# johannes-graeter/limo

Hardware: NVIDIA H100
Metric: BA windows/s (30 KF, 3k LM, 40k obs) (higher is better)
Workload: dtype f64

## Files before the change

### limo_b200/csrc/kba_api.cu

```cuda
#include <algorithm>
#include <atomic>
#include <chrono>
#include <cstdio>
#include <cstdlib>
#include <cstring>
#include <string>
#include <thread>
#include <vector>

#include <cuda_runtime.h>

#include "kba_b200.h"
#include "kba_kernels.h"

using namespace kba;

static thread_local std::string g_last_error;
static thread_local bool g_force_host_pack = false;
static int fail(int code, const std::string& msg) {
    g_last_error = msg;
    return code;
}
#define CU(call)                                                                                              \
    do {                                                                                                      \
// ... 576 lines not shown
        d.scale_kf0 = w[i].scale_kf0; d.scale_kf1 = w[i].scale_kf1;
        d.scale_weight = w[i].scale_weight; d.scale_value = w[i].scale_value;
        const bool planes = w[i].n_gp > 0 || w[i].plane_reg_weight > 0;
        const int rows = (planes ? 10 : 6) * w[i].n_kf + 1;
        max_rows = std::max(max_rows, rows);
        d.nr_cap = ((rows + 63) / 64) * 64;
        d.plane_reg_weight = w[i].plane_reg_weight; d.plane_dist_fixed = w[i].plane_dist_fixed;
        d.s_off = soff;
        soff += (long long)d.nr_cap * d.nr_cap;
        nr_cap_max = std::max(nr_cap_max, d.nr_cap);
        kf += w[i].n_kf; cam += w[i].n_cam; lm += w[i].n_lm; obs += w[i].n_obs; chunks += d.n_chunks; gp += w[i].n_gp;
        bd.max_obs = std::max(bd.max_obs, w[i].n_obs); bd.max_lm = std::max(bd.max_lm, w[i].n_lm);
        bd.max_kf = std::max(bd.max_kf, w[i].n_kf); bd.max_gp = std::max(bd.max_gp, w[i].n_gp);
    }
    if (obs > 2000000000LL) { b->release(); delete b; return fail(KBA_ERR_CAPACITY, "batch exceeds 2^31 observations"); }
    if (nr_cap_max > 640) {
        b->release();
        delete b;
        return fail(KBA_ERR_CAPACITY, "reduced system larger than 640 rows (106 keyframes, or 63 with ground-plane blocks)");
    }
    bd.tot_kf = kf; bd.tot_cam = cam; bd.tot_lm = lm; bd.tot_obs = obs; bd.tot_chunks = (int)chunks; bd.tot_gp = gp;
    bd.tot_groups = (int)groups;
    bd.nr_cap_max = nr_cap_max;
    b->lc.nr_cap_max = nr_cap_max;
    b->lc.sm_count = h->sm_count;
    {
        const int nb = nr_cap_max / 64, pairs = nb * (nb + 1) / 2;
        int max_chunks = 1;
        for (auto& d : b->desc_h) max_chunks = std::max(max_chunks, d.n_chunks);
        int p = std::min(16, (6 * h->sm_count + n_windows * pairs - 1) / (n_windows * pairs));
        b->lc.small_syrk = (max_rows <= 184);
        if (b->lc.small_syrk) p = (h->sm_count + n_windows - 1) / n_windows;
        bd.p_split = std::max(1, std::min(p, max_chunks));
        const char* fe = std::getenv("KBA_FUSED");
        bd.fused = (b->lc.small_syrk && bd.max_kf <= kFusedMaxKf && !(fe && std::atoi(fe) == 0)) ? 1 : 0;
        if (const char* pe = std::getenv("KBA_P_SPLIT")) { if (std::atoi(pe) > 0) p = std::atoi(pe); }
        if (bd.fused) bd.p_split = std::max(1, std::min(p, max_groups));
        else if (std::getenv("KBA_P_SPLIT")) bd.p_split = std::max(1, std::min(p, max_chunks));
        b->lc.fused_slots = (max_rows_free <= 176) ? 6 : 7;
    }
    bd.cost_parts = std::max((bd.max_obs + 255) / 256, (bd.max_obs / 16 + bd.max_lm / 32 + 4 + 7) / 8);
    { const char* le = std::getenv("KBA_LINEARIZE"); b->lc.lin_fused = !(le && std::atoi(le) == 0); }
    { const char* le = std::getenv("KBA_LIN_GRID"); if (le) b->lc.lin_grid = std::max(-1, std::atoi(le)); }
    { const char* le = std::getenv("KBA_BS_GRID"); if (le) b->lc.bs_grid = std::max(-1, std::atoi(le)); }
    {
        auto knob = [](const char* name, int dflt) { const char* e = std::getenv(name); return e ? std::atoi(e) : dflt; };
        bd.eval_tiles_jac = std::max(1, knob("KBA_EVAL_TILES_JAC", 8));
        bd.eval_tiles_cost = std::max(1, knob("KBA_EVAL_TILES_COST", 8));
        bd.eval_min_blocks = knob("KBA_EVAL_MIN_BLOCKS", 2);
        bd.eval_cs = knob("KBA_EVAL_CS", 0);
        bd.solve_row_major = knob("KBA_SOLVE_ROW_MAJOR", 0);
        bd.solve_tiled = (nr_cap_max <= 192 && !bd.solve_row_major) ? 1 : 0;
        const int split_dflt = (!bd.solve_tiled && n_windows <= 16) ? std::max(1, std::min(32, h->sm_count / n_windows)) : 0;
        bd.solve_split = bd.solve_tiled ? 0 : knob("KBA_SOLVE_SPLIT", split_dflt);
    }
    bd.bs_parts = (bd.max_lm + 15) / 16;
    {
        const char* pe = std::getenv("KBA_DEVICE_PACK");
        b->device_pack = bd.fused && !g_force_host_pack && bd.max_lm <= pack_max_landmarks() && !(pe && std::atoi(pe) == 0);
    }
    const bool hp = !b->device_pack;
    int bad = 0;
    bad |= b->desc.alloc(n_windows, true);
    bad |= b->pose0.alloc(7 * kf, true); bad |= b->plane0.alloc(4 * kf, true); bad |= b->kf_fixed.alloc(kf, true);
    bad |= b->cam.alloc(kCamStride * cam, true);
    bad |= b->lm0.alloc(3 * lm, hp); bad |= b->lm_weight.alloc(lm, hp); bad |= b->lm_ptr.alloc(lm + n_windows, hp);
    bad |= b->obs_kf.alloc(obs, hp); bad |= b->obs_cam.alloc(obs, hp); bad |= b->obs_lm.alloc(obs, hp);
    bad |= b->obs_u.alloc(obs, hp); bad |= b->obs_v.alloc(obs, hp); bad |= b->obs_d.alloc(obs, hp);
    bad |= b->kf_ptr.alloc(kf + n_windows, hp); bad |= b->pm_lm.alloc(obs, hp); bad |= b->pm_cam.alloc(obs, hp);
    bad |= b->pm_u.alloc(obs, hp); bad |= b->pm_v.alloc(obs, hp); bad |= b->pm_d.alloc(obs, hp);
    bad |= b->chunk_lm0.alloc(chunks, hp); bad |= b->chunk_lm1.alloc(chunks, hp);
    bad |= b->chunk_k0.alloc(chunks, hp); bad |= b->chunk_k1.alloc(chunks, hp);
    bad |= b->lm_orig.alloc(lm, hp); bad |= b->obs_rank.alloc(obs, hp);
    if (hp) bad |= b->obs_orig.alloc(obs, true);
    bad |= b->grp_k0.alloc(groups, hp); bad |= b->grp_k1.alloc(groups, hp);
    if (b->device_pack) {
        bad |= b->r_lm_ptr.alloc(lm + n_windows, true); bad |= b->r_obs_kf.alloc(obs, true); bad |= b->r_obs_cam.alloc(obs, true);
        bad |= b->r_obs_u.alloc(obs, true); bad |= b->r_obs_v.alloc(obs, true); bad |= b->r_obs_d.alloc(obs, true);
        bad |= b->r_lm_pos.alloc(3 * lm, true); bad |= b->r_lm_weight.alloc(lm, true); bad |= b->r_gp_lm.alloc(gp, true);
        bad |= b->lm_user.alloc(3 * lm, true); bad |= b->rej_user.alloc(lm, true);
        bad |= b->dev_alloc(&b->raw.lm_inv, lm);
    }
    bad |= b->dev_alloc(&bd.grp_t0, groups); bad |= b->dev_alloc(&bd.grp_t1, groups); bad |= b->dev_alloc(&bd.grp_rs, groups);
    bad |= b->dev_alloc(&bd.lin_tile, (size_t)(obs / 16) + (size_t)(lm / 32) + 4 * (size_t)n_windows + 4);
#ifdef KBA_PROF
    bad |= b->dev_alloc(&bd.prof, 16);
    if (!bad) cudaMemset(bd.prof, 0, 16 * sizeof(unsigned long long));
#endif
    bad |= b->dev_alloc(&bd.rt[0], (size_t)kPoseStride * kf); bad |= b->dev_alloc(&bd.rt[1], (size_t)kPoseStride * kf);
    {
        bd.panel_cap = 0;
        bd.vpanel = nullptr;
        bad |= b->dev_alloc(&bd.chunk_poff, chunks); bad |= b->dev_alloc(&bd.chunk_rs, chunks);
    }
    bad |= b->dev_alloc(&bd.chunk_t0, chunks); bad |= b->dev_alloc(&bd.chunk_t1, chunks); bad |= b->dev_alloc(&bd.obs_row, obs);
    bad |= b->state.alloc(n_windows, true); bad |= b->log.alloc((size_t)n_windows * kIterLogCap, true);
    for (int q = 0; q < 2; ++q) { bad |= b->pose_out[q].alloc(7 * kf, true); bad |= b->lm_out[q].alloc(3 * lm, hp); }
    bad |= b->lm_active.alloc(lm, hp); bad |= b->n_active.alloc(1, true); bad |= b->jac_obs.alloc(1, true);
    bad |= b->plane_out[0].alloc(4 * kf, true); bad |= b->plane_out[1].alloc(4 * kf, true);
    bad |= b->gp_lm.alloc(gp, hp); bad |= b->gp_kf.alloc(gp, true); bad |= b->gp_weight.alloc(gp, true); bad |= b->gp_of_lm.alloc(lm, hp); bad |= b->gp_shared.alloc(gp, hp);
    bad |= b->dev_alloc(&bd.gp_lin, 14 * gp); bad |= b->dev_alloc(&bd.vgp, 30 * gp);
    bad |= b->dev_alloc(&bd.gp_cost_x, n_windows); bad |= b->dev_alloc(&bd.gp_cost_c, n_windows);
    bad |= b->dev_alloc(&bd.off_pose, kf); bad |= b->dev_alloc(&bd.off_dir, kf); bad |= b->dev_alloc(&bd.off_dist, kf);
    bad |= b->dev_alloc(&bd.bkf, 27 * kf);
    bad |= b->dev_alloc(&bd.scale_f, (size_t)n_windows * nr_cap_max); bad |= b->dev_alloc(&bd.lambda_f, (size_t)n_windows * nr_cap_max);
    bad |= b->dev_alloc(&bd.grad_f, (size_t)n_windows * nr_cap_max); bad |= b->dev_alloc(&bd.delta_f, (size_t)n_windows * nr_cap_max);
    bad |= b->dev_alloc(&bd.lm_scale, 3 * lm); bad |= b->dev_alloc(&bd.lm_linv, 6 * lm); bad |= b->dev_alloc(&bd.lm_z, 3 * lm);
    bad |= b->dev_alloc(&bd.lm_g, 3 * lm); bad |= b->dev_alloc(&bd.lm_lambda, 3 * lm); bad |= b->dev_alloc(&bd.trim_val, 3 * lm);
    bad |= b->dev_alloc(&bd.trim_reject, lm);
    bad |= b->dev_alloc(&bd.res, 3 * obs); bad |= b->dev_alloc(&bd.jp, 18 * obs);
    if (!bd.fused) bad |= b->dev_alloc(&bd.jl, 9 * obs);
    else { bad |= b->dev_alloc(&bd.vobs, 18 * obs); bad |= b->dev_alloc(&bd.lm_run, lm); }
    bad |= b->dev_alloc(&bd.cost_part_x, (size_t)n_windows * bd.cost_parts); bad |= b->dev_alloc(&bd.cost_part_c, (size_t)n_windows * bd.cost_parts);
    bad |= b->dev_alloc(&bd.bs_part, (size_t)n_windows * bd.bs_parts * 4);
    bad |= b->dev_alloc(&bd.sred, (size_t)soff * bd.p_split); bad |= b->dev_alloc(&bd.amat, (size_t)soff);
    bad |= b->dev_alloc(&bd.chol_w, (size_t)n_windows * 32 * 32); bad |= b->dev_alloc(&bd.chol_invd, (size_t)n_windows * nr_cap_max);
    if (bad) {
        const std::string msg = std::string("device/pinned allocation failed: ") + cudaGetErrorString(cudaGetLastError());
        b->release(); delete b;
        return fail(KBA_ERR_CUDA, msg);
    }
    bd.desc = b->desc.d; bd.state = b->state.d; bd.log = b->log.d;
    bd.pose0 = b->pose0.d; bd.plane0 = b->plane0.d; bd.pose[0] = b->pose_out[0].d; bd.pose[1] = b->pose_out[1].d;
    bd.kf_fixed = b->kf_fixed.d; bd.cam = b->cam.d;
    bd.lm0 = b->lm0.d; bd.lm[0] = b->lm_out[0].d; bd.lm[1] = b->lm_out[1].d; bd.lm_weight = b->lm_weight.d;
    bd.lm_active = b->lm_active.d; bd.lm_ptr = b->lm_ptr.d;
    bd.obs_kf = b->obs_kf.d; bd.obs_cam = b->obs_cam.d; bd.obs_lm = b->obs_lm.d;
    bd.obs_u = b->obs_u.d; bd.obs_v = b->obs_v.d; bd.obs_d = b->obs_d.d;
    bd.kf_ptr = b->kf_ptr.d; bd.pm_lm = b->pm_lm.d; bd.pm_cam = b->pm_cam.d; bd.pm_u = b->pm_u.d; bd.pm_v = b->pm_v.d; bd.pm_d = b->pm_d.d;
    bd.chunk_lm0 = b->chunk_lm0.d; bd.chunk_lm1 = b->chunk_lm1.d; bd.chunk_k0 = b->chunk_k0.d; bd.chunk_k1 = b->chunk_k1.d;
    bd.lm_orig = b->lm_orig.d;
    bd.obs_rank = b->obs_rank.d;
    bd.grp_k0 = b->grp_k0.d; bd.grp_k1 = b->grp_k1.d;
    bd.plane[0] = b->plane_out[0].d; bd.plane[1] = b->plane_out[1].d;
    bd.gp_lm = b->gp_lm.d; bd.gp_kf = b->gp_kf.d; bd.gp_weight = b->gp_weight.d; bd.gp_of_lm = b->gp_of_lm.d; bd.gp_shared = b->gp_shared.d;
    bd.n_active = b->n_active.d;
    bd.jac_obs = b->jac_obs.d;
    if (b->device_pack) {
        PackRaw& r = b->raw;
        r.lm_ptr = b->r_lm_ptr.d; r.obs_kf = b->r_obs_kf.d; r.obs_cam = b->r_obs_cam.d;
        r.obs_u = b->r_obs_u.d; r.obs_v = b->r_obs_v.d; r.obs_d = b->r_obs_d.d;
        r.lm_pos = b->r_lm_pos.d; r.lm_weight = b->r_lm_weight.d; r.gp_lm = b->r_gp_lm.d; r.obs_orig = nullptr;
    }
    {
        cudaError_t e = cudaMemset(bd.jac_obs, 0, sizeof(unsigned long long));
        if (e == cudaSuccess) e = cudaEventCreate(&b->ev_a);
        if (e == cudaSuccess) e = cudaEventCreate(&b->ev_b);
        if (e == cudaSuccess) e = cudaEventCreateWithFlags(&b->ev_poll, (h->blocking_sync ? cudaEventBlockingSync : 0) | cudaEventDisableTiming);
        if (e == cudaSuccess) e = cudaEventCreateWithFlags(&b->ev_poll2, (h->blocking_sync ? cudaEventBlockingSync : 0) | cudaEventDisableTiming);
        if (e == cudaSuccess && b->loop_pass.alloc(1, true)) e = cudaErrorMemoryAllocation;
        if (e == cudaSuccess) e = configure_kernels(nr_cap_max);
        if (e == cudaSuccess && b->device_pack) e = configure_pack();
        if (e != cudaSuccess) { b->release(); delete b; return fail(KBA_ERR_CUDA, cudaGetErrorString(e)); }
    }
    *out = b;
    const int rc = kba_batch_upload(b, n_windows, w);
    if (rc != KBA_OK) { b->release(); delete b; *out = nullptr; }
    return rc;
}

int kba_batch_upload(kba_batch* b, int32_t n_windows, const kba_window* w) {
    if (!b || !w || n_windows != b->bd.n_win) return fail(KBA_ERR_BAD_ARG, "bad argument to kba_batch_upload");
    CU(cudaSetDevice(b->h->device));
    for (int i = 0; i < n_windows; ++i) {
        const WinDesc& d = b->desc_h[i];
        std::string why;
// ... 695 lines not shown
```

### limo_b200/csrc/kba_device.cuh

```cuda
#pragma once
#include <cstdint>
#include <cuda_runtime.h>

namespace kba {

constexpr int kMaxKf = 128;
constexpr int kMaxCam = 8;
constexpr int kPoseStride = 12;
constexpr int kCamStride = 16;
constexpr int kIterLogCap = 160;
constexpr int kFusedMaxKf = 32;

struct WinDesc {
    int n_kf, n_cam, n_lm, n_obs, n_gp;
    int kf_off, cam_off, lm_off, obs_off, gp_off;
    int chunk_off, n_chunks;
    int grp_off, n_groups;
    int scale_kf0, scale_kf1;
    double scale_weight, scale_value;
    double plane_reg_weight;
    int plane_dist_fixed, landmarks_fixed;
    int speed_kf, pad0;
    double speed_weight, speed_dt;
    double speed_v_before[3];
// ... 55 lines not shown
    double* plane0;
    double* pose[2];
    double* rt[2];
    double* plane[2];
    uint8_t* kf_fixed;
    int* off_pose;
    int* off_dir;
    int* off_dist;
    double* bkf;
    double* scale_f;
    double* cam;
    double* lm0;
    double* lm[2];
    double* lm_weight;
    uint8_t* lm_active;
    uint8_t* lm_active0;
    int* lm_ptr;
    double* lm_scale;
    double* lm_linv;
    double* lm_z;
    double* lm_g;
    double* lm_lambda;
    double* trim_val;
    uint8_t* trim_reject;
    int* obs_kf;
    int* obs_cam;
    int* obs_lm;
    int* obs_rank;
    float* obs_u, *obs_v, *obs_d;
    int* kf_ptr;
    int* pm_lm;
    int* pm_cam;
    float* pm_u, *pm_v, *pm_d;
    double* res;
    double* jp;
    double* jl;
    double* vpanel;
    long long panel_cap;
    int* chunk_poff;
    int* chunk_rs;
    double* cost_part_x;
    double* cost_part_c;
    int cost_parts;
    int sharded;
    int lm_begin, lm_total;
    int shard_rank, shard_world;
    double* xs;
    double* x_send;
    double* x_recv;
    double* trim_send;
    double* trim_glob;
    uint8_t* reject_glob;
    int precision;
    int solve_row_major;
    int solve_tiled;
    int solve_split;
    double* chol_w;
    double* chol_invd;
    int eval_tiles_jac, eval_tiles_cost, eval_min_blocks;
    int eval_cs;
    double* bs_part;
    int bs_parts;
    int nr_cap_max;
    double* sred;
    int p_split;
    double* delta_f;
    double* lambda_f;
    double* grad_f;
    double* amat;
    int* chunk_lm0;
    int* chunk_lm1;
    int* chunk_k0;
    int* chunk_k1;
    int* chunk_t0;
    int* chunk_t1;
    int* obs_row;
    int* lm_orig;
    int tot_chunks;
    int fused;
    int* grp_k0;
    int* grp_k1;
    int* grp_t0;
    int* grp_t1;
    int* grp_rs;
    double* vobs;
    int4* lm_run;
    int lin1;
    int2* lin_tile;
    unsigned long long* prof;
    int tot_groups;
    int* n_active;
    unsigned long long* jac_obs;
    int* gp_lm;
    int* gp_kf;
    double* gp_weight;
    int* gp_of_lm;
    int* gp_shared;
    double* gp_lin;
    double* vgp;
    double* gp_cost_x;
    double* gp_cost_c;
};

struct SolveParams {
    double gp_huber, gp_quantile;
    double depth_thres, reprojection_thres, depth_quantile, reprojection_quantile;
    double function_tolerance, gradient_tolerance, parameter_tolerance;
    double initial_radius, max_radius, min_radius, min_relative_decrease, min_lm_diagonal, max_lm_diagonal;
    int trim_solver_iterations, final_solver_iterations, min_residual_groups, max_consecutive_invalid_steps;
    double max_solver_time;
};

__device__ __forceinline__ unsigned long long global_timer_ns() {
    unsigned long long t;
    asm volatile("mov.u64 %0, %%globaltimer;" : "=l"(t));
    return t;
}

template <typename T>
__host__ __device__ inline void quat_to_rot(const T* q, T* R) {
    const T w = q[0], x = q[1], y = q[2], z = q[3];
    const T tx = 2 * x, ty = 2 * y, tz = 2 * z;
    const T twx = tx * w, twy = ty * w, twz = tz * w, txx = tx * x, txy = ty * x, txz = tz * x;
    const T tyy = ty * y, tyz = tz * y, tzz = tz * z;
    R[0] = 1 - (tyy + tzz); R[1] = txy - twz;       R[2] = txz + twy;
    R[3] = txy + twz;       R[4] = 1 - (txx + tzz); R[5] = tyz - twx;
    R[6] = txz - twy;       R[7] = tyz + twx;       R[8] = 1 - (txx + tyy);
}

__host__ __device__ inline void pose_plus(const double* p, const double* d, double* o) {
    const double nd = sqrt(d[0] * d[0] + d[1] * d[1] + d[2] * d[2]);
    if (nd > 0.0) {
        const double s = sin(nd) / nd, c = cos(nd);
        const double q0 = c, q1 = s * d[0], q2 = s * d[1], q3 = s * d[2];
        o[0] = q0 * p[0] - q1 * p[1] - q2 * p[2] - q3 * p[3];
        o[1] = q0 * p[1] + q1 * p[0] + q2 * p[3] - q3 * p[2];
        o[2] = q0 * p[2] - q1 * p[3] + q2 * p[0] + q3 * p[1];
        o[3] = q0 * p[3] + q1 * p[2] - q2 * p[1] + q3 * p[0];
    } else {
        o[0] = p[0]; o[1] = p[1]; o[2] = p[2]; o[3] = p[3];
    }
    o[4] = p[4] + d[3]; o[5] = p[5] + d[4]; o[6] = p[6] + d[5];
}

template <typename T, bool kCost = true>
__device__ inline void cauchy(T b, T w, T s, T& half_rho, T& sqrt_rho1) {
    const T sum = T(1) + s / b;
    half_rho = kCost ? T(0.5) * w * b * log(sum) : T(0);
    sqrt_rho1 = sqrt(w / sum);
}

template <typename T, bool kM, bool kCost = true>
__device__ __forceinline__ bool eval_factored(const T* __restrict__ pose, const T* __restrict__ cam, const T p[3], T u, T v,
                                              T d, T wt, T b_repr, T b_depth, T r[3], T m[9], T a[3], T& half_rho_sum,
                                              T raw[2]) {
    a[0] = pose[0] * p[0] + pose[1] * p[1] + pose[2] * p[2];
    a[1] = pose[3] * p[0] + pose[4] * p[1] + pose[5] * p[2];
    a[2] = pose[6] * p[0] + pose[7] * p[1] + pose[8] * p[2];
    const T x0 = a[0] + pose[9], x1 = a[1] + pose[10], x2 = a[2] + pose[11];
    const T c0 = cam[0] * x0 + cam[1] * x1 + cam[2] * x2 + cam[9];
    const T c1 = cam[3] * x0 + cam[4] * x1 + cam[5] * x2 + cam[10];
    const T c2 = cam[6] * x0 + cam[7] * x1 + cam[8] * x2 + cam[11];
    if (!(fabs(c2) >= T(0.01))) return false;
    const bool has_d = d > T(0);
    const T rd = has_d ? c2 - d : T(0);
    const T f = cam[12], iz = T(1) / c2;
// ... 202 lines not shown
```

### limo_b200/csrc/kba_kernels.cu

```cuda
#include "kba_device.cuh"
#include "kba_kernels.h"
#include "kba_regularisers.cuh"
#include "kba_prep.cuh"
#include "kba_linearize.cuh"

#include <cfloat>
#include <cstdio>
#include <cstdlib>
#include <cmath>
#include <type_traits>

namespace kba {

constexpr int kBeginThreads = 1024;
__global__ void __launch_bounds__(kBeginThreads) k_solve_begin(BatchDev bd, SolveParams sp) {
    const int w = blockIdx.x;
    WinState& st = bd.state[w];
    if (st.phase != PH_SOLVE_BEGIN) return;
    const WinDesc wd = bd.desc[w];
    __shared__ int s_has[kMaxKf];
    __shared__ int s_plane[kMaxKf];
    __shared__ int s_cnt[3];
    __shared__ int s_tile_chunk[513];
    for (int k = threadIdx.x; k < wd.n_kf; k += blockDim.x) { s_has[k] = 0; s_plane[k] = 0; }
// ... 38 lines not shown
            bd.off_pose[wd.kf_off + k] = var ? n : -1;
            if (var) n += 6;
            const bool pl = (s_plane[k] || chain) && !fixed;
            bd.off_dir[wd.kf_off + k] = pl ? n : -1;
            if (pl) n += 3;
            const bool pd = pl && !wd.plane_dist_fixed;
            bd.off_dist[wd.kf_off + k] = pd ? n : -1;
            if (pd) n += 1;
        }
        if (chain) n_reg = 3 * (wd.n_kf - 1) + wd.n_kf;
        st.n_f = n;
        st.nr = (n + 1 + 7) & ~7;
        st.radius = sp.initial_radius;
        st.decrease_factor = 2.0;
        st.iteration = 0;
        st.num_invalid = 0;
        st.last_successful = 0;
        st.need_linearize = 1;
        st.iter0 = 1;
        st.eval_failed = 0;
        st.solve_failed = 0;
        st.max_iter = st.is_final ? sp.final_solver_iterations
                                  : (st.retried ? 3 * sp.trim_solver_iterations : sp.trim_solver_iterations);
        SolveSummary& s = st.solves[st.solve_index];
        s.initial_cost = s.final_cost = 0.0;
        s.num_iterations = 0; s.num_successful_steps = 0; s.termination = 1;
        s.num_landmarks = s_cnt[0];
        s.num_residual_blocks = s_cnt[1] + s_cnt[2] + n_reg + (wd.scale_weight > 0 ? 1 : 0) + (wd.speed_weight > 0 ? 1 : 0);
        st.t_solve_start = global_timer_ns();
        st.phase = PH_ITERATE;
    }
    __syncthreads();
    for (int o = threadIdx.x; o < wd.n_obs; o += blockDim.x) {
        const size_t oo = (size_t)wd.obs_off + o;
        const bool act = bd.lm_active[wd.lm_off + bd.obs_lm[oo]];
        bd.obs_row[oo] = act ? bd.off_pose[wd.kf_off + bd.obs_kf[oo]] : -1;
    }
    for (int c = threadIdx.x; c < (bd.fused ? 0 : wd.n_chunks); c += blockDim.x) {
        int r0 = 1 << 30, r1 = -1;
        for (int k = bd.chunk_k0[wd.chunk_off + c]; k <= bd.chunk_k1[wd.chunk_off + c]; ++k) {
            const int off = bd.off_pose[wd.kf_off + k], od = bd.off_dir[wd.kf_off + k], oz = bd.off_dist[wd.kf_off + k];
            if (off >= 0) { r0 = min(r0, off); r1 = max(r1, off + 6); }
            if (od >= 0) { r0 = min(r0, od); r1 = max(r1, od + 3); }
            if (oz >= 0) { r0 = min(r0, oz); r1 = max(r1, oz + 1); }
        }
        bd.chunk_t0[wd.chunk_off + c] = (r1 < 0) ? 0 : r0 / 8;
        bd.chunk_t1[wd.chunk_off + c] = (r1 < 0) ? 0 : (r1 + 7) / 8;
    }
    if (bd.fused) {
        __syncthreads();
        for (int j = threadIdx.x; j < wd.n_lm; j += blockDim.x) {
            const int o0 = lm_ptr[j], o1 = lm_ptr[j + 1];
            int n_start = 0, n_valid = 0, bad = 0, a = 0, row_a = 0, prev = -2;
            for (int o = o0; o < o1; ++o) {
                const size_t oo = (size_t)wd.obs_off + o;
                const int r = bd.obs_row[oo];
                if (r >= 0) {
                    ++n_valid;
                    if (prev < 0) { if (n_start++ == 0) { a = o - o0; row_a = r; } }
                    else if (r != prev + 6) bad = 1;
                    if (bd.obs_rank[oo] != 0) bad = 1;
                }
                prev = r;
            }
            int4 run = make_int4(0, 0, 0, 0);
            if (n_valid > 0) run = (bad || n_start != 1) ? make_int4(0, -1, 0, 0) : make_int4(a, n_valid, row_a, 0);
            bd.lm_run[wd.lm_off + j] = run;
        }
    }
    if (bd.fused) build_lin_tiles(bd, wd, st, w, s_tile_chunk);
    if (bd.fused) {
        const int trhs = st.n_f >> 3;
        for (int c = threadIdx.x; c < wd.n_groups; c += blockDim.x) {
            int r0 = 1 << 30, r1 = -1;
            for (int k = bd.grp_k0[wd.grp_off + c]; k <= bd.grp_k1[wd.grp_off + c]; ++k) {
                const int off = bd.off_pose[wd.kf_off + k], od = bd.off_dir[wd.kf_off + k], oz = bd.off_dist[wd.kf_off + k];
                if (off >= 0) { r0 = min(r0, off); r1 = max(r1, off + 6); }
                if (od >= 0) { r0 = min(r0, od); r1 = max(r1, od + 3); }
                if (oz >= 0) { r0 = min(r0, oz); r1 = max(r1, oz + 1); }
            }
            const int t0 = (r1 < 0) ? 0 : (r0 / 16) * 2, t1 = (r1 < 0) ? 0 : ((r1 + 15) / 16) * 2;
            int rows = 0;
            if (t1 > t0) rows = 8 * (t1 - t0) + ((trhs >= t0 && trhs < t1) ? 0 : 8);
            bd.grp_t0[wd.grp_off + c] = t0;
            bd.grp_t1[wd.grp_off + c] = t1;
            bd.grp_rs[wd.grp_off + c] = rows;
        }
    }
    if (!bd.fused) {
        __syncthreads();
        if (threadIdx.x == 0) {
            const int trhs = st.n_f >> 3;
            int poff = 0;
            for (int c = 0; c < wd.n_chunks; ++c) {
                const int t0 = bd.chunk_t0[wd.chunk_off + c], t1 = bd.chunk_t1[wd.chunk_off + c];
                int rs = 0;
                if (t1 > t0) {
                    const int rows = 8 * (t1 - t0) + ((trhs >= t0 && trhs < t1) ? 0 : 8);
                    rs = ((rows - 4 + 15) / 16) * 16 + 4;
                }
                bd.chunk_rs[wd.chunk_off + c] = rs;
                bd.chunk_poff[wd.chunk_off + c] = poff;
                poff += 96 * rs;
            }
        }
    }
}

__global__ void __launch_bounds__(256) k_panel_zero(BatchDev bd) {
    const int w = blockIdx.y;
    if (bd.fused || bd.state[w].phase != PH_SOLVE_BEGIN || bd.desc[w].landmarks_fixed) return;
    double2* p = reinterpret_cast<double2*>(bd.vpanel + bd.desc[w].panel_off);
    const long long n2 = bd.panel_cap / 2;
    for (long long i = (long long)blockIdx.x * blockDim.x + threadIdx.x; i < n2; i += (long long)gridDim.x * blockDim.x)
        p[i] = make_double2(0.0, 0.0);
}

template <bool kJac, int kMinBlocks, typename TLin, bool kJl = true, bool kCs = false>
__global__ void __launch_bounds__(256, kMinBlocks) k_eval_obs(BatchDev bd, SolveParams sp, int tiles) {
    const int w = blockIdx.y;
    WinState& st = bd.state[w];
    const WinDesc& wd = bd.desc[w];
    const int n_obs = wd.n_obs, obs_off = wd.obs_off, lm_off = wd.lm_off;
    if (st.phase != PH_ITERATE) return;
    if (kJac && !st.need_linearize) return;
    if (!kJac && st.solve_failed) return;
    __shared__ __align__(16) double s_pose[kMaxKf * kPoseStride];
    __shared__ __align__(16) double s_cam[kMaxCam * kCamStride];
    __shared__ __align__(8) uint64_t s_bar;
    __shared__ double s_red[8];
    __shared__ int s_cnt[8];
    constexpr bool kF32 = sizeof(TLin) == 4;
    __shared__ float s_pose_f[kF32 ? kMaxKf * kPoseStride : 1];
    __shared__ float s_cam_f[kF32 ? kMaxCam * kCamStride : 1];
    const int buf = kJac ? st.cur : 1 - st.cur;
    const double* __restrict__ lm_buf = bd.lm[buf];
    const int i0 = blockIdx.x * tiles * 256 + threadIdx.x;
    int idx_b = (i0 < n_obs) ? bd.obs_lm[(size_t)obs_off + i0] : -1;
    int idx_a = (tiles > 1 && i0 + 256 < n_obs) ? bd.obs_lm[(size_t)obs_off + i0 + 256] : -1;
    int L = -1, kfi = 0, cami = 0, row = -1;
    float u = 0.f, v = 0.f, d = 0.f;
    double p0 = 0, p1 = 0, p2 = 0, wgt = 0;
    unsigned char act = 0;
    if (idx_b >= 0) {
        const size_t o = (size_t)obs_off + i0;
        L = lm_off + idx_b;
        kfi = bd.obs_kf[o]; cami = bd.obs_cam[o];
        if (kJac) row = bd.obs_row[o];
        u = bd.obs_u[o]; v = bd.obs_v[o]; d = bd.obs_d[o];
        p0 = lm_buf[3 * (size_t)L]; p1 = lm_buf[3 * (size_t)L + 1]; p2 = lm_buf[3 * (size_t)L + 2];
        wgt = bd.lm_weight[L];
        act = bd.lm_active[L];
    }
    stage_window_bulk(wd, bd.rt[buf], bd.cam, s_pose, s_cam, &s_bar);
    if (kF32) {
        for (int i = threadIdx.x; i < wd.n_kf * kPoseStride; i += blockDim.x) s_pose_f[i] = (float)s_pose[i];
        for (int i = threadIdx.x; i < wd.n_cam * kCamStride; i += blockDim.x) s_cam_f[i] = (float)s_cam[i];
        __syncthreads();
    }
    double cost = 0.0;
    int done = 0;
#pragma unroll 1
    for (int t = 0; t < tiles; ++t) {
        const int i_n = i0 + (t + 1) * 256;
        int Ln = -1, kfn = 0, camn = 0, rown = -1;
        float un = 0.f, vn = 0.f, dn = 0.f;
        double q0 = 0, q1 = 0, q2 = 0, wn = 0;
        unsigned char actn = 0;
// ... 2065 lines not shown
```

### limo_b200/csrc/kba_schur_fused.cuh

```cuda
#pragma once

namespace kba {

constexpr int kLG = 8;
constexpr int kGC = 3 * kLG;
constexpr int kFStages = 6;
constexpr int kFMaxRs = 196;
constexpr int kFStageDoubles = kGC * kFMaxRs;
constexpr int kFObs = 128;
constexpr int kFConsumerWarps = 12;
constexpr int kFMaxKf = 32;

__constant__ signed char kSyrkMap12[12][7] = {
    {72, 7, 22, 33, 36, 48, 65}, {67, 10, 12, 19, 40, 53, -1}, {73, 1, 13, 17, 42, 50, -1}, {77, 8, 21, 26, 39, 54, -1},
    {75, 3, 18, 34, 49, 57, -1}, {69, 6, 23, 41, 58, 62, -1},  {66, 11, 27, 32, 38, 64, -1}, {74, 9, 20, 30, 37, 52, 55},
    {68, 0, 14, 16, 31, 44, 51}, {76, 2, 24, 29, 43, 45, 60},  {71, 5, 25, 28, 46, 56, 63},  {70, 4, 15, 35, 47, 59, 61}};

__device__ __forceinline__ void mbar_arrive(uint64_t* bar) {
    asm volatile("mbarrier.arrive.shared::cta.b64 _, [%0];" ::"r"(smem_u32(bar)) : "memory");
}
__device__ __forceinline__ void cp_async_elem(double* dst, const double* src) {
    asm volatile("cp.async.ca.shared.global [%0], [%1], 8;" ::"r"(smem_u32(dst)), "l"(src) : "memory");
}
__device__ __forceinline__ void cp_async_elem(float* dst, const float* src) {
    asm volatile("cp.async.ca.shared.global [%0], [%1], 4;" ::"r"(smem_u32(dst)), "l"(src) : "memory");
}
__device__ __forceinline__ void cp_async16(double* dst, const double* src) {
    asm volatile("cp.async.cg.shared.global [%0], [%1], 16;" ::"r"(smem_u32(dst)), "l"(src) : "memory");
}
__device__ __forceinline__ void cp_async8(double* dst, const double* src) {
    asm volatile("cp.async.ca.shared.global [%0], [%1], 8;" ::"r"(smem_u32(dst)), "l"(src) : "memory");
}
__device__ __forceinline__ void cp_async_arrive(uint64_t* bar) {
    asm volatile("cp.async.mbarrier.arrive.noinc.shared::cta.b64 [%0];" ::"r"(smem_u32(bar)) : "memory");
}
__device__ __forceinline__ void cp_async_commit() { asm volatile("cp.async.commit_group;" ::: "memory"); }
template <int N>
__device__ __forceinline__ void cp_async_wait() { asm volatile("cp.async.wait_group %0;" ::"n"(N) : "memory"); }
__device__ __forceinline__ void producer_sync() { asm volatile("bar.sync 1, 128;" ::: "memory"); }
template <int N>
__device__ __forceinline__ void reg_dec() { asm volatile("setmaxnreg.dec.sync.aligned.u32 %0;" ::"n"(N)); }
template <int N>
__device__ __forceinline__ void reg_inc() { asm volatile("setmaxnreg.inc.sync.aligned.u32 %0;" ::"n"(N)); }

constexpr size_t schur_fused_smem() { return (size_t)kFStages * kFStageDoubles * sizeof(double) + 24 * sizeof(uint64_t); }

#ifdef KBA_PROF
#define KBA_PROF_DECL long long pt_ = clock64(), pacc_[3] = {0, 0, 0}
#define KBA_PROF_T0 pt_ = clock64()
#define KBA_PROF_ACC(i) do { const long long n_ = clock64(); pacc_[i] += n_ - pt_; pt_ = n_; } while (0)
#define KBA_PROF_FLUSH(base) do { if (lane == 0 && bd.prof) for (int i_ = 0; i_ < 3; ++i_) atomicAdd(bd.prof + (base) + i_, (unsigned long long)pacc_[i_]); } while (0)
#else
#define KBA_PROF_DECL
#define KBA_PROF_T0
#define KBA_PROF_ACC(i)
#define KBA_PROF_FLUSH(base)
#endif

__device__ __forceinline__ void schur_split(int n_groups, int p_split, int& per, int& used) {
    per = max(8, (n_groups + p_split - 1) / p_split);
    used = max(1, min(p_split, (n_groups + per - 1) / per));
}

template <int kSlots>
__global__ void __launch_bounds__(512, 1) k_schur_fused(BatchDev bd) {
    const int w = blockIdx.y;
    const WinState& st = bd.state[w];
    if (st.phase != PH_ITERATE || st.solve_failed) return;
    const WinDesc& wd = bd.desc[w];
    if (wd.landmarks_fixed) return;
    extern __shared__ __align__(128) unsigned char fsm[];
    double* stage = reinterpret_cast<double*>(fsm);
    uint64_t* full = reinterpret_cast<uint64_t*>(fsm + (size_t)kFStages * kFStageDoubles * sizeof(double));
    uint64_t* empty = full + kFStages;
    const int tid = threadIdx.x, warp = tid >> 5, lane = tid & 31;
    const int n_f = st.n_f, nt = (n_f + 8) >> 3, trhs = n_f >> 3;
    int per, used;
    schur_split(wd.n_groups, (int)gridDim.x, per, used);
    if ((int)blockIdx.x >= used) return;
    const int g0 = blockIdx.x * per, g1 = min(wd.n_groups, g0 + per);
    const int* grs = bd.grp_rs + wd.grp_off;
    const int* gt0 = bd.grp_t0 + wd.grp_off;
    const int* gt1 = bd.grp_t1 + wd.grp_off;
    if (tid == 0) {
        for (int i = 0; i < kFStages; ++i) { mbar_init(&full[i], 1); mbar_init(&empty[i], kFConsumerWarps); }
        asm volatile("fence.proxy.async.shared::cta;" ::: "memory");
    }
    __syncthreads();
    auto next_group = [&](int g) { while (g < g1 && grs[g] == 0) ++g; return g; };

    if (warp >= kFConsumerWarps) {
        if (kSlots == 7) reg_dec<56>(); else reg_dec<104>();

        const int pw = warp - kFConsumerWarps;
        const int* lm_ptr = bd.lm_ptr + wd.lm_off + w;
        const size_t base = (size_t)wd.obs_off, TG = (size_t)bd.tot_gp;
        const bool sync_path = wd.n_gp > 0 || wd.max_rank > 0;
        const int cj = lane / 3, cc = lane - 3 * cj;
        const int zj = lane - 24;
        int g1_ = -1, rs1 = 0, t01 = 0, t11 = 0, act1 = 0, p01 = 0, p11 = 0;
        int4 run1 = make_int4(0, 0, 0, 0);
        KBA_PROF_DECL;
        auto load_meta = [&](int g) {
            g1_ = g; act1 = 0; run1 = make_int4(0, 0, 0, 0); p01 = p11 = 0;
            if (g >= g1) return;
            rs1 = grs[g]; t01 = gt0[g]; t11 = gt1[g];
            if (lane < 24) {
                const int j = g * kLG + cj;
                if (j < wd.n_lm) { run1 = bd.lm_run[wd.lm_off + j]; p01 = lm_ptr[j]; p11 = lm_ptr[j + 1]; }
            } else {
                const int j = g * kLG + zj;
                if (j < wd.n_lm) { act1 = bd.lm_active[wd.lm_off + j]; p01 = lm_ptr[j]; p11 = lm_ptr[j + 1]; }
            }
        };
        auto nth_group = [&](int g, int n) {
            g = next_group(g);
            for (; n > 0 && g < g1; --n) g = next_group(g + 1);
            return g;
        };
        int g = nth_group(g0, pw), gi = pw;
        load_meta(g);
        while (g < g1) {
            const int rs = rs1, t0 = t01, t1 = t11, act0 = act1, p00 = p01, p10 = p11;
            const int4 run0 = run1;
            const int gnext = nth_group(g + 1, 3);
            load_meta(gnext);
            const int slot = gi % kFStages;
            KBA_PROF_T0;
            if (gi >= kFStages) mbar_wait(&empty[slot], ((gi / kFStages) - 1) & 1);
            KBA_PROF_ACC(0);
            double* sb = stage + (size_t)slot * kFStageDoubles;
            {
                const int h = rs >> 1;
                for (int c = 0; c < kGC; ++c)
                    for (int r2 = lane; r2 < h; r2 += 32) reinterpret_cast<double2*>(sb + (size_t)c * kFMaxRs)[r2] = make_double2(0.0, 0.0);
            }
            const bool no_run = lane < 24 && (run0.y < 0 || (run0.y > 0 && ((run0.z - 8 * t0) & 1)));
            const bool bulk = __ballot_sync(0xffffffffu, no_run) == 0u && !sync_path;
            asm volatile("fence.proxy.async.shared::cta;" ::: "memory");
            __syncwarp();
            KBA_PROF_ACC(1);
            const int j0 = g * kLG, j1 = min(wd.n_lm, j0 + kLG);
            const int ob = lm_ptr[j0], oe = lm_ptr[j1];
            const int rl = (trhs >= t0 && trhs < t1) ? n_f - 8 * t0 : 8 * (t1 - t0) + (n_f - 8 * trhs);
            if (bulk) {
                if (lane < 24 && run0.y > 0) {
                    const uint32_t bytes = (uint32_t)(48 * run0.y);
                    asm volatile("mbarrier.expect_tx.relaxed.cta.shared::cta.b64 [%0], %1;" ::"r"(smem_u32(&full[slot])), "r"(bytes) : "memory");
                    tma_load_1d(sb + (size_t)(3 * cj + cc) * kFMaxRs + (run0.z - 8 * t0),
                                bd.vobs + vobs_index(base, p00, p10, p00 + run0.x, cc), bytes, &full[slot]);
                }
            } else {
                for (int o = ob + lane; o < oe; o += 32) {
                    const size_t oo = base + o;
                    const int row = bd.obs_row[oo];
                    if (row < 0 || bd.obs_rank[oo] != 0) continue;
                    const int lm = bd.obs_lm[oo], q0 = lm_ptr[lm], q1 = lm_ptr[lm + 1];
                    double* dst = sb + (size_t)(3 * (lm - j0)) * kFMaxRs + (row - 8 * t0);
#pragma unroll
                    for (int c = 0; c < 3; ++c) {
                        const double* src = bd.vobs + vobs_index(base, q0, q1, o, c);
                        if (((row - 8 * t0) & 1) == 0) {
#pragma unroll
                            for (int h = 0; h < 3; ++h) cp_async16(dst + c * kFMaxRs + 2 * h, src + 2 * h);
                        } else {
#pragma unroll
                            for (int r = 0; r < 6; ++r) cp_async8(dst + c * kFMaxRs + r, src + r);
                        }
                    }
                }
            }
            if (lane >= 24 && act0 && p10 > p00) {
                const double* zz = bd.lm_z + 3 * (size_t)(wd.lm_off + j0 + zj);
                double* col = sb + (size_t)(3 * zj) * kFMaxRs + rl;
                cp_async8(col, zz); cp_async8(col + kFMaxRs, zz + 1); cp_async8(col + 2 * kFMaxRs, zz + 2);
            }
            if (!sync_path) {
                asm volatile("cp.async.mbarrier.arrive.shared::cta.b64 [%0];" ::"r"(smem_u32(&full[slot])) : "memory");
                __syncwarp();
                if (lane == 0) mbar_arrive(&full[slot]);
            } else {
                cp_async_commit();
                cp_async_wait<0>();
                __syncwarp();
                for (int round = 1; round <= wd.max_rank; ++round) {
                    for (int o = ob + lane; o < oe; o += 32) {
                        const size_t oo = base + o;
                        const int row = bd.obs_row[oo];
                        if (row < 0 || bd.obs_rank[oo] != round) continue;
                        const int lm = bd.obs_lm[oo], q0 = lm_ptr[lm], q1 = lm_ptr[lm + 1];
                        double* dst = sb + (size_t)(3 * (lm - j0)) * kFMaxRs + (row - 8 * t0);
                        for (int c = 0; c < 3; ++c) {
                            const double* src = bd.vobs + vobs_index(base, q0, q1, o, c);
                            for (int r = 0; r < 6; ++r) dst[c * kFMaxRs + r] += src[r];
                        }
                    }
                    __syncwarp();
                }
                if (wd.n_gp > 0) {
                    for (int it = lane; it < 80; it += 32) {
                        const int jj = it / 10, r = it - 10 * jj, j = j0 + jj;
                        const int L = wd.lm_off + j;
                        if (j >= wd.n_lm || !bd.lm_active[L] || lm_ptr[j + 1] <= lm_ptr[j]) continue;
                        const int gl = bd.gp_of_lm[L];
                        if (gl < 0) continue;
                        const size_t G = (size_t)wd.gp_off + gl;
                        const int row = gp_row(bd, wd, bd.gp_kf[G], r);
                        if (row < 0) continue;
                        double* q = sb + (size_t)(3 * jj) * kFMaxRs + (row - 8 * t0);
                        q[0] += bd.vgp[(3 * r + 0) * TG + G];
                        q[kFMaxRs] += bd.vgp[(3 * r + 1) * TG + G];
                        q[2 * kFMaxRs] += bd.vgp[(3 * r + 2) * TG + G];
                    }
                }
                __syncwarp();
                if (lane == 0) mbar_arrive(&full[slot]);
            }
            KBA_PROF_ACC(2);
            g = gnext; gi += 4;
        }
        cp_async_commit();
        cp_async_wait<0>();
        KBA_PROF_FLUSH(4);
        return;
    }

    if (kSlots == 7) reg_inc<152>(); else reg_inc<136>();
    const int fr = lane >> 2, fc = lane & 3;
    const int nb2 = (nt + 1) >> 1, brhs = trhs >> 1;
    double acc[kSlots][4][2];
    int my_bi[kSlots], my_bj[kSlots];
#pragma unroll
    for (int s = 0; s < kSlots; ++s) {
#pragma unroll
        for (int q = 0; q < 4; ++q) acc[s][q][0] = acc[s][q][1] = 0.0;
        const int t = kSyrkMap12[warp][s + (7 - kSlots)];
        int bi = 1 << 20, bj = 0;
        if (t >= 0) {
            bi = (int)((sqrtf(8.0f * (float)t + 1.0f) - 1.0f) * 0.5f);
            while ((bi + 1) * (bi + 2) / 2 <= t) ++bi;
            while (bi * (bi + 1) / 2 > t) --bi;
            bj = t - bi * (bi + 1) / 2;
        }
        if (bi >= nb2) bi = 1 << 20;
        my_bi[s] = bi; my_bj[s] = bj;
    }
    {
        int gi = 0;
        int g = next_group(g0), t0 = 0, t1 = 0;
        if (g < g1) { t0 = gt0[g]; t1 = gt1[g]; }
        KBA_PROF_DECL;
        for (; g < g1; ++gi) {
            const int gn = next_group(g + 1);
            int t0n = 0, t1n = 0;
            if (gn < g1) { t0n = gt0[gn]; t1n = gt1[gn]; }
            const int slot = gi % kFStages;
            KBA_PROF_T0;
            mbar_wait(&full[slot], (gi / kFStages) & 1);
            KBA_PROF_ACC(0);
            const int b0 = t0 >> 1, b1 = t1 >> 1;
            const bool rhs_in = brhs >= b0 && brhs < b1;
            const int rhs_row = 16 * (b1 - b0);
            const double* sb = stage + (size_t)slot * kFStageDoubles + (size_t)fc * kFMaxRs + fr;
#pragma unroll
            for (int s = 0; s < kSlots; ++s) {
                const int bi = my_bi[s], bj = my_bj[s];
                if (bj < b0 || bj >= b1) continue;
                if (bi >= b0 && bi < b1) {
                    const double* pa = sb + 16 * (bi - b0);
                    const double* pb = sb + 16 * (bj - b0);
                    if (bi != bj) {
#pragma unroll
                        for (int kk = 0; kk < kGC; kk += 4) {
                            const double a0 = pa[kk * kFMaxRs], a1 = pa[kk * kFMaxRs + 8], b0v = pb[kk * kFMaxRs], b1v = pb[kk * kFMaxRs + 8];
                            dmma(acc[s][0][0], acc[s][0][1], a0, b0v);
                            dmma(acc[s][1][0], acc[s][1][1], a0, b1v);
                            dmma(acc[s][2][0], acc[s][2][1], a1, b0v);
                            dmma(acc[s][3][0], acc[s][3][1], a1, b1v);
                        }
                    } else {
#pragma unroll
                        for (int kk = 0; kk < kGC; kk += 4) {
                            const double a0 = pa[kk * kFMaxRs], a1 = pa[kk * kFMaxRs + 8];
                            dmma(acc[s][0][0], acc[s][0][1], a0, a0);
                            dmma(acc[s][2][0], acc[s][2][1], a1, a0);
                            dmma(acc[s][3][0], acc[s][3][1], a1, a1);
                        }
                    }
                } else if (bi == brhs && !rhs_in) {
                    const double* pa = sb + rhs_row;
                    const double* pb = sb + 16 * (bj - b0);
                    if (trhs & 1) {
#pragma unroll
                        for (int kk = 0; kk < kGC; kk += 4) {
                            const double a1 = pa[kk * kFMaxRs], b0v = pb[kk * kFMaxRs], b1v = pb[kk * kFMaxRs + 8];
                            dmma(acc[s][2][0], acc[s][2][1], a1, b0v);
                            dmma(acc[s][3][0], acc[s][3][1], a1, b1v);
                        }
                    } else {
#pragma unroll
                        for (int kk = 0; kk < kGC; kk += 4) {
                            const double a0 = pa[kk * kFMaxRs], b0v = pb[kk * kFMaxRs], b1v = pb[kk * kFMaxRs + 8];
                            dmma(acc[s][0][0], acc[s][0][1], a0, b0v);
                            dmma(acc[s][1][0], acc[s][1][1], a0, b1v);
                        }
                    }
                }
            }
            __syncwarp();
            if (lane == 0) mbar_arrive(&empty[slot]);
            KBA_PROF_ACC(1);
            g = gn; t0 = t0n; t1 = t1n;
        }
        KBA_PROF_FLUSH(0);
    }
    double* out = bd.sred + wd.s_off * (size_t)bd.p_split + (size_t)blockIdx.x * wd.nr_cap * wd.nr_cap;
#pragma unroll
    for (int s = 0; s < kSlots; ++s) {
        const int bi = my_bi[s], bj = my_bj[s];
        if (bi >= nb2) continue;
#pragma unroll
        for (int q = 0; q < 4; ++q) {
            const int i = 2 * bi + (q >> 1), j = 2 * bj + (q & 1);
            if (i >= nt || j > i) continue;
            double* o = out + (size_t)(8 * i + fr) * wd.nr_cap + 8 * j + 2 * fc;
            o[0] = acc[s][q][0];
            o[1] = acc[s][q][1];
        }
    }
}

}
```

Baseline: 1333.

## Use m16n8 f64 MMA with column-half skipping in fused Schur SYRK

Reworks the consumer-warp SYRK in the fused Schur kernel to use m16n8k4/k8 double-precision MMA instead of m8n8k4. Each 16x16 block pair is now computed as two 16x8 halves, and halves that fall outside the group's actual 8-row extent are skipped. That extent is packed per group in a new grp_tiles array. The block map is precomputed as packed nibbles, replacing the sqrt-based decoding, and register budgets are unified. This aims to cut wasted MMA work and instruction count, at the cost of a changed accumulator layout and more template instantiation and code size.

Measured after the change: 1409, median of 6. 5.7% higher.

```diff
diff --git a/limo_b200/csrc/kba_api.cu b/limo_b200/csrc/kba_api.cu
--- a/limo_b200/csrc/kba_api.cu
+++ b/limo_b200/csrc/kba_api.cu
@@ -682,6 +682,7 @@
         bad |= b->dev_alloc(&b->raw.lm_inv, lm);
     }
     bad |= b->dev_alloc(&bd.grp_t0, groups); bad |= b->dev_alloc(&bd.grp_t1, groups); bad |= b->dev_alloc(&bd.grp_rs, groups);
+    bad |= b->dev_alloc(&bd.grp_tiles, groups);
     bad |= b->dev_alloc(&bd.lin_tile, (size_t)(obs / 16) + (size_t)(lm / 32) + 4 * (size_t)n_windows + 4);
 #ifdef KBA_PROF
     bad |= b->dev_alloc(&bd.prof, 16);
diff --git a/limo_b200/csrc/kba_device.cuh b/limo_b200/csrc/kba_device.cuh
--- a/limo_b200/csrc/kba_device.cuh
+++ b/limo_b200/csrc/kba_device.cuh
@@ -161,6 +161,7 @@
     int* grp_k1;
     int* grp_t0;
     int* grp_t1;
+    int* grp_tiles;
     int* grp_rs;
     double* vobs;
     int4* lm_run;
diff --git a/limo_b200/csrc/kba_kernels.cu b/limo_b200/csrc/kba_kernels.cu
--- a/limo_b200/csrc/kba_kernels.cu
+++ b/limo_b200/csrc/kba_kernels.cu
@@ -144,8 +144,15 @@
             const int t0 = (r1 < 0) ? 0 : (r0 / 16) * 2, t1 = (r1 < 0) ? 0 : ((r1 + 15) / 16) * 2;
             int rows = 0;
             if (t1 > t0) rows = 8 * (t1 - t0) + ((trhs >= t0 && trhs < t1) ? 0 : 8);
+            int e0 = 0, e1 = 0;
+            if (t1 > t0) {
+                e0 = r0 / 8;
+                e1 = (r1 + 7) / 8;
+                if (trhs >= t0 && trhs < t1) e1 = max(e1, trhs + 1);
+            }
             bd.grp_t0[wd.grp_off + c] = t0;
             bd.grp_t1[wd.grp_off + c] = t1;
+            bd.grp_tiles[wd.grp_off + c] = t0 | t1 << 8 | e0 << 16 | e1 << 24;
             bd.grp_rs[wd.grp_off + c] = rows;
         }
     }
diff --git a/limo_b200/csrc/kba_schur_fused.cuh b/limo_b200/csrc/kba_schur_fused.cuh
--- a/limo_b200/csrc/kba_schur_fused.cuh
+++ b/limo_b200/csrc/kba_schur_fused.cuh
@@ -11,10 +11,11 @@
 constexpr int kFConsumerWarps = 12;
 constexpr int kFMaxKf = 32;
 
-__constant__ signed char kSyrkMap12[12][7] = {
-    {72, 7, 22, 33, 36, 48, 65}, {67, 10, 12, 19, 40, 53, -1}, {73, 1, 13, 17, 42, 50, -1}, {77, 8, 21, 26, 39, 54, -1},
-    {75, 3, 18, 34, 49, 57, -1}, {69, 6, 23, 41, 58, 62, -1},  {66, 11, 27, 32, 38, 64, -1}, {74, 9, 20, 30, 37, 52, 55},
-    {68, 0, 14, 16, 31, 44, 51}, {76, 2, 24, 29, 43, 45, 60},  {71, 5, 25, 28, 46, 56, 63},  {70, 4, 15, 35, 47, 59, 61}};
+__constant__ unsigned char kSyrkMap12[12][7] = {
+    {0xb6, 0x31, 0x61, 0x75, 0x80, 0x93, 0xaa}, {0xb1, 0x40, 0x42, 0x54, 0x84, 0x98, 0xff}, {0xb7, 0x10, 0x43, 0x52, 0x86, 0x95, 0xff},
+    {0xbb, 0x32, 0x60, 0x65, 0x83, 0x99, 0xff}, {0xb9, 0x20, 0x53, 0x76, 0x94, 0xa2, 0xff}, {0xb3, 0x30, 0x62, 0x85, 0xa3, 0xa7, 0xff},
+    {0xb0, 0x41, 0x66, 0x74, 0x82, 0xa9, 0xff}, {0xb8, 0x33, 0x55, 0x72, 0x81, 0x97, 0xa0}, {0xb2, 0x00, 0x44, 0x51, 0x73, 0x88, 0x96},
+    {0xba, 0x11, 0x63, 0x71, 0x87, 0x90, 0xa5}, {0xb5, 0x22, 0x64, 0x70, 0x91, 0xa1, 0xa8}, {0xb4, 0x21, 0x50, 0x77, 0x92, 0xa4, 0xa6}};
 
 __device__ __forceinline__ void mbar_arrive(uint64_t* bar) {
     asm volatile("mbarrier.arrive.shared::cta.b64 _, [%0];" ::"r"(smem_u32(bar)) : "memory");
@@ -60,6 +61,53 @@
 __device__ __forceinline__ void schur_split(int n_groups, int p_split, int& per, int& used) {
     per = max(8, (n_groups + p_split - 1) / p_split);
     used = max(1, min(p_split, (n_groups + per - 1) / per));
+}
+
+__device__ __forceinline__ void dmma16k4(double (&c)[4], double a0, double a1, double b0) {
+    asm volatile("mma.sync.aligned.m16n8k4.row.col.f64.f64.f64.f64 {%0,%1,%2,%3}, {%4,%5}, {%6}, {%0,%1,%2,%3};\n"
+                 : "+d"(c[0]), "+d"(c[1]), "+d"(c[2]), "+d"(c[3])
+                 : "d"(a0), "d"(a1), "d"(b0));
+}
+__device__ __forceinline__ void dmma16k8(double (&c)[4], double a0, double a1, double a2, double a3, double b0, double b1) {
+    asm volatile("mma.sync.aligned.m16n8k8.row.col.f64.f64.f64.f64 {%0,%1,%2,%3}, {%4,%5,%6,%7}, {%8,%9}, {%0,%1,%2,%3};\n"
+                 : "+d"(c[0]), "+d"(c[1]), "+d"(c[2]), "+d"(c[3])
+                 : "d"(a0), "d"(a1), "d"(a2), "d"(a3), "d"(b0), "d"(b1));
+}
+
+template <bool kL, bool kR, bool kRhs, bool kK8>
+__device__ __forceinline__ void syrk_block(double (&c)[2][4], const double* pa, const double* pb, bool odd) {
+    if (kK8 && !kRhs) {
+#pragma unroll
+        for (int kk = 0; kk < kGC; kk += 8) {
+            const double* qa = pa + kk * kFMaxRs;
+            const double* qb = pb + kk * kFMaxRs;
+            const double a0 = qa[0], a1 = qa[8], a2 = qa[4 * kFMaxRs], a3 = qa[4 * kFMaxRs + 8];
+            if (kL) dmma16k8(c[0], a0, a1, a2, a3, qb[0], qb[4 * kFMaxRs]);
+            if (kR) dmma16k8(c[1], a0, a1, a2, a3, qb[8], qb[4 * kFMaxRs + 8]);
+        }
+    } else {
+#pragma unroll
+        for (int kk = 0; kk < kGC; kk += 4) {
+            double a0, a1;
+            if (kRhs) {
+                const double a = pa[kk * kFMaxRs];
+                a0 = odd ? 0.0 : a;
+                a1 = odd ? a : 0.0;
+            } else {
+                a0 = pa[kk * kFMaxRs];
+                a1 = pa[kk * kFMaxRs + 8];
+            }
+            if (kL) dmma16k4(c[0], a0, a1, pb[kk * kFMaxRs]);
+            if (kR) dmma16k4(c[1], a0, a1, pb[kk * kFMaxRs + 8]);
+        }
+    }
+}
+
+template <bool kRhs, bool kK8>
+__device__ __forceinline__ void syrk_halves(double (&c)[2][4], const double* pa, const double* pb, bool odd, bool lo, bool hi) {
+    if (lo && hi) syrk_block<true, true, kRhs, kK8>(c, pa, pb, odd);
+    else if (lo) syrk_block<true, false, kRhs, kK8>(c, pa, pb, odd);
+    else if (hi) syrk_block<false, true, kRhs, kK8>(c, pa, pb, odd);
 }
 
 template <int kSlots>
@@ -82,6 +130,7 @@
     const int* grs = bd.grp_rs + wd.grp_off;
     const int* gt0 = bd.grp_t0 + wd.grp_off;
     const int* gt1 = bd.grp_t1 + wd.grp_off;
+    const int* gtl = bd.grp_tiles + wd.grp_off;
     if (tid == 0) {
         for (int i = 0; i < kFStages; ++i) { mbar_init(&full[i], 1); mbar_init(&empty[i], kFConsumerWarps); }
         asm volatile("fence.proxy.async.shared::cta;" ::: "memory");
@@ -90,7 +139,7 @@
     auto next_group = [&](int g) { while (g < g1 && grs[g] == 0) ++g; return g; };
 
     if (warp >= kFConsumerWarps) {
-        if (kSlots == 7) reg_dec<56>(); else reg_dec<104>();
+        reg_dec<56>();
 
         const int pw = warp - kFConsumerWarps;
         const int* lm_ptr = bd.lm_ptr + wd.lm_off + w;
@@ -225,109 +274,63 @@
         return;
     }
 
-    if (kSlots == 7) reg_inc<152>(); else reg_inc<136>();
+    reg_inc<152>();
     const int fr = lane >> 2, fc = lane & 3;
     const int nb2 = (nt + 1) >> 1, brhs = trhs >> 1;
-    double acc[kSlots][4][2];
-    int my_bi[kSlots], my_bj[kSlots];
-#pragma unroll
-    for (int s = 0; s < kSlots; ++s) {
-#pragma unroll
-        for (int q = 0; q < 4; ++q) acc[s][q][0] = acc[s][q][1] = 0.0;
-        const int t = kSyrkMap12[warp][s + (7 - kSlots)];
-        int bi = 1 << 20, bj = 0;
-        if (t >= 0) {
-            bi = (int)((sqrtf(8.0f * (float)t + 1.0f) - 1.0f) * 0.5f);
-            while ((bi + 1) * (bi + 2) / 2 <= t) ++bi;
-            while (bi * (bi + 1) / 2 > t) --bi;
-            bj = t - bi * (bi + 1) / 2;
-        }
-        if (bi >= nb2) bi = 1 << 20;
-        my_bi[s] = bi; my_bj[s] = bj;
-    }
+    double acc[kSlots][2][4];
+    const unsigned char* my_b = kSyrkMap12[warp] + (7 - kSlots);
+#pragma unroll
+    for (int s = 0; s < kSlots; ++s)
+#pragma unroll
+        for (int q = 0; q < 4; ++q) acc[s][0][q] = acc[s][1][q] = 0.0;
     {
         int gi = 0;
-        int g = next_group(g0), t0 = 0, t1 = 0;
-        if (g < g1) { t0 = gt0[g]; t1 = gt1[g]; }
+        int g = next_group(g0), tiles = 0;
+        if (g < g1) tiles = gtl[g];
         KBA_PROF_DECL;
         for (; g < g1; ++gi) {
             const int gn = next_group(g + 1);
-            int t0n = 0, t1n = 0;
-            if (gn < g1) { t0n = gt0[gn]; t1n = gt1[gn]; }
+            const int tiles_n = gn < g1 ? gtl[gn] : 0;
             const int slot = gi % kFStages;
             KBA_PROF_T0;
             mbar_wait(&full[slot], (gi / kFStages) & 1);
             KBA_PROF_ACC(0);
-            const int b0 = t0 >> 1, b1 = t1 >> 1;
+            const int b0 = (tiles & 255) >> 1, b1 = ((tiles >> 8) & 255) >> 1;
+            const int e0 = (tiles >> 16) & 255, e1 = tiles >> 24;
             const bool rhs_in = brhs >= b0 && brhs < b1;
             const int rhs_row = 16 * (b1 - b0);
             const double* sb = stage + (size_t)slot * kFStageDoubles + (size_t)fc * kFMaxRs + fr;
 #pragma unroll
             for (int s = 0; s < kSlots; ++s) {
-                const int bi = my_bi[s], bj = my_bj[s];
+                const int b = my_b[s], bi = b >> 4, bj = b & 15;
                 if (bj < b0 || bj >= b1) continue;
-                if (bi >= b0 && bi < b1) {
-                    const double* pa = sb + 16 * (bi - b0);
-                    const double* pb = sb + 16 * (bj - b0);
-                    if (bi != bj) {
-#pragma unroll
-                        for (int kk = 0; kk < kGC; kk += 4) {
-                            const double a0 = pa[kk * kFMaxRs], a1 = pa[kk * kFMaxRs + 8], b0v = pb[kk * kFMaxRs], b1v = pb[kk * kFMaxRs + 8];
-                            dmma(acc[s][0][0], acc[s][0][1], a0, b0v);
-                            dmma(acc[s][1][0], acc[s][1][1], a0, b1v);
-                            dmma(acc[s][2][0], acc[s][2][1], a1, b0v);
-                            dmma(acc[s][3][0], acc[s][3][1], a1, b1v);
-                        }
-                    } else {
-#pragma unroll
-                        for (int kk = 0; kk < kGC; kk += 4) {
-                            const double a0 = pa[kk * kFMaxRs], a1 = pa[kk * kFMaxRs + 8];
-                            dmma(acc[s][0][0], acc[s][0][1], a0, a0);
-                            dmma(acc[s][2][0], acc[s][2][1], a1, a0);
-                            dmma(acc[s][3][0], acc[s][3][1], a1, a1);
-                        }
-                    }
-                } else if (bi == brhs && !rhs_in) {
-                    const double* pa = sb + rhs_row;
-                    const double* pb = sb + 16 * (bj - b0);
-                    if (trhs & 1) {
-#pragma unroll
-                        for (int kk = 0; kk < kGC; kk += 4) {
-                            const double a1 = pa[kk * kFMaxRs], b0v = pb[kk * kFMaxRs], b1v = pb[kk * kFMaxRs + 8];
-                            dmma(acc[s][2][0], acc[s][2][1], a1, b0v);
-                            dmma(acc[s][3][0], acc[s][3][1], a1, b1v);
-                        }
-                    } else {
-#pragma unroll
-                        for (int kk = 0; kk < kGC; kk += 4) {
-                            const double a0 = pa[kk * kFMaxRs], b0v = pb[kk * kFMaxRs], b1v = pb[kk * kFMaxRs + 8];
-                            dmma(acc[s][0][0], acc[s][0][1], a0, b0v);
-                            dmma(acc[s][1][0], acc[s][1][1], a0, b1v);
-                        }
-                    }
-                }
+                const bool lo = 2 * bj >= e0, hi = 2 * bj + 1 < e1;
+                const double* pb = sb + 16 * (bj - b0);
+                if (bi == bj) syrk_halves<false, kSlots == 6>(acc[s], pb, pb, false, lo, hi);
+                else if (bi >= b0 && bi < b1) syrk_halves<false, kSlots == 6>(acc[s], sb + 16 * (bi - b0), pb, false, lo, hi);
+                else if (bi == brhs && !rhs_in) syrk_halves<true, false>(acc[s], sb + rhs_row, pb, trhs & 1, lo, hi);
             }
             __syncwarp();
             if (lane == 0) mbar_arrive(&empty[slot]);
             KBA_PROF_ACC(1);
-            g = gn; t0 = t0n; t1 = t1n;
+            g = gn; tiles = tiles_n;
         }
         KBA_PROF_FLUSH(0);
     }
     double* out = bd.sred + wd.s_off * (size_t)bd.p_split + (size_t)blockIdx.x * wd.nr_cap * wd.nr_cap;
 #pragma unroll
     for (int s = 0; s < kSlots; ++s) {
-        const int bi = my_bi[s], bj = my_bj[s];
+        const int b = my_b[s], bi = b >> 4, bj = b & 15;
         if (bi >= nb2) continue;
 #pragma unroll
         for (int q = 0; q < 4; ++q) {
             const int i = 2 * bi + (q >> 1), j = 2 * bj + (q & 1);
             if (i >= nt || j > i) continue;
             double* o = out + (size_t)(8 * i + fr) * wd.nr_cap + 8 * j + 2 * fc;
-            o[0] = acc[s][q][0];
-            o[1] = acc[s][q][1];
-        }
-    }
-}
-
-}
+            o[0] = acc[s][q & 1][2 * (q >> 1)];
+            o[1] = acc[s][q & 1][2 * (q >> 1) + 1];
+        }
+    }
+}
+
+}
```
